# So-bonkers/Detecting-Convolutional-Codes-Via-Markovian-Statistics

Hardware: AMD Instinct MI355X
Metric: MC trials/sec at N=1e5, rate-1/2 m=6 pair, 1/2/4/8 GPUs; Pd match vs CPU (higher is better)
Workload: dtype u32 bit-planes (metrics, four planes of the 64 states) + f64 (log-likelihood sums)

## Files before the change

__graft_entry__.py:

```python
import importlib.util
import os
import subprocess
import sys

ROOT = os.path.dirname(os.path.abspath(__file__))
PKG_DIR = os.path.join(ROOT, "detecting-convolutional-codes-via-markovian-statistics_amd")
PKG_NAME = "dccvm_amd"


def load_package():
    if PKG_NAME in sys.modules:
        return sys.modules[PKG_NAME]
    spec = importlib.util.spec_from_file_location(
        PKG_NAME, os.path.join(PKG_DIR, "__init__.py"), submodule_search_locations=[PKG_DIR])
    mod = importlib.util.module_from_spec(spec)
    sys.modules[PKG_NAME] = mod
    spec.loader.exec_module(mod)
    return mod


def build() -> None:
    jobs = str(min(16, os.cpu_count() or 4))
    subprocess.check_call(["make", "-j", jobs, "-C", os.path.join(PKG_DIR, "csrc")])
    subprocess.check_call(["make", "-C", os.path.join(ROOT, "oracle")])
# ... 2 lines not shown
    prebuild_jit(pkg, lib)


def prebuild_jit(pkg, lib, arch="gfx950"):
    import ctypes
    jit_dir = os.path.join(PKG_DIR, "lib", "jit")
    so_time = os.path.getmtime(os.path.join(PKG_DIR, "lib", "libcvd.so"))
    if os.path.isdir(jit_dir):
        old = [f for f in os.listdir(jit_dir) if f.endswith(".co")]
        if any(os.path.getmtime(os.path.join(jit_dir, f)) < so_time for f in old):
            for f in old:
                os.remove(os.path.join(jit_dir, f))
    for name, cc in pkg.CONFIG_CODES.items():
        code = pkg.Code(cc["gen1"], cc["m"], cc["k"], cc["n"])
        n = ctypes.c_int32(0)
        rc = lib.cvd_jit_prebuild(code.c, arch.encode(), jit_dir.encode(), ctypes.byref(n))
        if rc != 0:
            print(f"jit prebuild of {name} failed: {lib.cvd_last_error().decode(errors='replace')}", file=sys.stderr)


def smoke() -> None:
    if ROOT not in sys.path:
        sys.path.insert(0, ROOT)
    pkg = load_package()
    from oracle import restatement as R
    k, n, m = 1, 2, 2
    g1 = [[[1, 1, 1]], [[1, 0, 1]]]
    g2 = [[[1, 0, 1]], [[1, 1, 1]]]
    N, p, seed, trials = 200, 0.1, 123, 64
    det = pkg.Detector(k, n, m, g1, device=0)
    model = det.model(p, learn_len=None, learn_burn=200, laplace=1.0, seed=seed)
    res = det.run_trials(model, g1, g2, N, p, seed, 0, trials, return_sums=True)
    states, transitions, all_r = R.enumerate_markov_states_allzero(g1, m, k, n)
# ... 36 lines not shown
```

detecting-convolutional-codes-via-markovian-statistics_amd/_lib.py:

```python
import ctypes
import os

import torch

_HERE = os.path.dirname(os.path.abspath(__file__))
LIB_PATH = os.environ.get("CVD_LIB_PATH") or os.path.join(_HERE, "lib", "libcvd.so")
ABI_VERSION = 11

PATH_AUTO, PATH_TABLE, PATH_EXPLICIT, PATH_EXPLICIT_GENERIC, PATH_EXPLICIT_ORBIT, PATH_EXPLICIT_BUTTERFLY = 0, 1, 2, 3, 4, 5
DETECT_EARLY_DECISION = 0x100
CAPTURE_LSB, CAPTURE_MSB, CAPTURE_BYTES = 0, 1, 2
CAPTURE_FORMATS = {"lsb": CAPTURE_LSB, "msb": CAPTURE_MSB, "bytes": CAPTURE_BYTES}


class CvdError(RuntimeError):
    """Raised when a libcvd call returns a negative status."""


class cvd_code(ctypes.Structure):
    _fields_ = [("k", ctypes.c_int32), ("n", ctypes.c_int32), ("m", ctypes.c_int32),
                ("taps", ctypes.POINTER(ctypes.c_uint8))]


class cvd_learn_params(ctypes.Structure):
# ... 73 lines not shown
    "cvd_mc_workspace_bytes": (ctypes.c_int64, [ctypes.POINTER(cvd_code), ctypes.c_int64, ctypes.c_int64]),
    "cvd_mc_run": (ctypes.c_int, [ctypes.c_void_p, ctypes.POINTER(cvd_code), ctypes.POINTER(cvd_code),
                                  ctypes.c_double, ctypes.c_int64, ctypes.c_uint64, ctypes.c_int64,
                                  ctypes.c_int64, ctypes.c_int64, ctypes.c_void_p, ctypes.c_void_p,
                                  ctypes.c_int32, ctypes.c_void_p]),
    "cvd_mc_grid_workspace_bytes": (ctypes.c_int64, [ctypes.c_void_p, ctypes.c_int32, ctypes.POINTER(cvd_code),
                                                     ctypes.c_void_p, ctypes.c_int32, ctypes.c_int64, ctypes.c_int32]),
    "cvd_mc_run_grid": (ctypes.c_int, [ctypes.c_void_p, ctypes.POINTER(cvd_code), ctypes.POINTER(cvd_code),
                                       ctypes.c_void_p, ctypes.c_int32, ctypes.c_void_p, ctypes.c_int32,
                                       ctypes.c_uint64, ctypes.c_int64, ctypes.c_int64, ctypes.c_int64,
                                       ctypes.c_void_p, ctypes.c_void_p, ctypes.c_int32, ctypes.c_void_p]),
    "cvd_model_device_error": (ctypes.c_int, [ctypes.c_void_p, ctypes.POINTER(ctypes.c_int32)]),
    "cvd_chunk_last": (ctypes.c_int, [ctypes.POINTER(ctypes.c_int64)]),
    "cvd_jit_prebuild": (ctypes.c_int, [ctypes.POINTER(cvd_code), ctypes.c_char_p, ctypes.c_char_p,
                                        ctypes.POINTER(ctypes.c_int32)]),
    "cvd_mc_fused": (ctypes.c_int, [ctypes.c_void_p, ctypes.POINTER(cvd_code), ctypes.POINTER(cvd_code),
                                    ctypes.c_double, ctypes.c_int64, ctypes.c_uint64, ctypes.c_int64,
                                    ctypes.c_int64, ctypes.c_void_p, ctypes.c_void_p, ctypes.c_int32,
                                    ctypes.c_void_p]),
    "cvd_parity_detect": (ctypes.c_int, [ctypes.c_void_p, ctypes.c_int32, ctypes.c_int64, ctypes.c_int64,
                                         ctypes.c_int64, ctypes.c_void_p, ctypes.c_int32, ctypes.c_double,
                                         ctypes.c_void_p, ctypes.c_void_p, ctypes.c_void_p]),
    "cvd_parity_sweep_workspace_bytes": (ctypes.c_int64, [ctypes.c_int32, ctypes.c_int32, ctypes.c_int32]),
    "cvd_parity_sweep": (ctypes.c_int, [ctypes.c_void_p, ctypes.c_int64, ctypes.c_int32, ctypes.c_int32,
                                        ctypes.c_int32, ctypes.c_int64, ctypes.c_int64, ctypes.c_int32,
                                        ctypes.c_void_p, ctypes.c_void_p, ctypes.c_void_p]),
    "cvd_viterbi_workspace_bytes": (ctypes.c_int64, [ctypes.c_int32, ctypes.c_int32, ctypes.c_int64, ctypes.c_int32]),
    "cvd_viterbi_decode": (ctypes.c_int, [ctypes.POINTER(cvd_code), ctypes.c_void_p, ctypes.c_int64, ctypes.c_int32,
                                          ctypes.c_int64, ctypes.c_int64, ctypes.c_int32, ctypes.c_int32,
                                          ctypes.c_int32, ctypes.c_void_p, ctypes.c_void_p, ctypes.c_void_p,
# ... 77 lines not shown
```

detecting-convolutional-codes-via-markovian-statistics_amd/csrc/cvd_host.cpp:

```cpp
#include <atomic>
#include <chrono>
#include <functional>
#include <map>
#include <mutex>
#include <thread>
#include <tuple>
#include <cstdlib>
#include <exception>
#include <cstdio>
#include <algorithm>
#include <cmath>
#include <cstring>
#include <memory>
#include <new>
#include <stdexcept>
#include <string>
#include <unordered_map>
#include <vector>

#include <sys/stat.h>
#include <unistd.h>

#include "../../include/cvd.h"
#include "cvd_internal.h"
// ... 1060 lines not shown
  const auto t0 = std::chrono::steady_clock::now();
  const int rc = model_create(dec, prm, device, stream, out, &st);
  st.seconds = std::chrono::duration<double>(std::chrono::steady_clock::now() - t0).count();
  if (stats_out) {
    stats_out[0] = st.seconds;
    stats_out[1] = (double)st.mismatched_blocks;
    stats_out[2] = (double)st.fix_passes;
    stats_out[3] = (double)st.sequential_blocks;
    stats_out[4] = (double)st.hash_attempts;
    stats_out[5] = (double)st.host_fallback;
    stats_out[6] = st.sequential_seconds;
  }
  return rc;
}

extern "C" int cvd_jit_prebuild(const cvd_code* dec, const char* arch, const char* dir, int32_t* n_built) {
  CVD_TRY
  if (!dec || !arch || !dir || !n_built) { set_error("null argument"); return CVD_E_INVALID; }
  *n_built = 0;
  cvd_model Mo;
  int rc = parse_code(dec, Mo.dec);
  if (rc) return rc;
  const Tabs T = make_tabs(Mo.dec);
  build_bmp(Mo, T);
  if (!Mo.k1b_ok || !bitslice_preferred(Mo)) return CVD_OK;
  const std::string vs[] = {
      rtc_variant_defs(kBsPfLog2Bits >= 20 ? 1024 : 512, false, kFilterPatBitsLds, true, true, kBsPfLog2Bits),
      rtc_variant_defs(1024, true, kFilterPatBitsLds, true, false, kBsPfLog2Bits),
      rtc_variant_defs(512, true, kFilterPatBitsLds, true, false, kBsPfLog2Bits)};
  std::vector<std::thread> th;
  std::vector<int> res(3, 0);
  std::vector<std::string> errs(3);
  for (int i = 0; i < 3; ++i)
    th.emplace_back([&, i] {
      res[i] = rtc_prebuild(Mo.dec.m, Mo.bfly_x, vs[i].c_str(), arch, dir);
      if (res[i]) errs[i] = last_error_copy();
    });
  for (auto& t : th) t.join();
  for (int i = 0; i < 3; ++i) {
    if (res[i]) { set_error(errs[i]); return CVD_E_UNSUPPORTED; }
    ++*n_built;
  }
  return CVD_OK;
  CVD_CATCH
}

extern "C" int cvd_model_info_get(const cvd_model* Mo, cvd_model_info* info) {
  if (!Mo || !info) { set_error("null argument"); return CVD_E_INVALID; }
  info->kind = Mo->kind;
  info->k = Mo->dec.k; info->n = Mo->dec.n; info->m = Mo->dec.m;
  info->S = Mo->S;
  info->n_rows = Mo->n_rows;
  info->learn_len_eff = Mo->learn_len_eff;
  info->hash_capacity = Mo->hcap;
  info->max_probe = Mo->max_probe;
  info->device = Mo->device;
  info->logp1_unseen = Mo->logp1_unseen;
  info->explicit_kernel = explicit_kernel_of(*Mo);
  info->mc_fused = mc_fused_preferred(*Mo) ? 1 : 0;
// ... 65 lines not shown
```

detecting-convolutional-codes-via-markovian-statistics_amd/csrc/cvd_internal.h:

```cpp
#pragma once
#include <stdint.h>

#include <array>
#include <string>
#include <vector>

#include "cvd_common.h"
#include "cvd_keys.h"

struct cvd_code;

struct cvd_model {
  cvd::CodeDesc dec;
  int32_t kind = 0;
  int64_t S = 0;
  int64_t learn_len_eff = 0;
  double laplace = 1.0;
  double logp1_unseen = 0.0;
  double lp_min = 0.0;
  std::vector<double> ltref;

  int64_t n_rows = 0;
  std::vector<uint8_t> keys;
  std::vector<double> logp1;
// ... 34 lines not shown
  int32_t slot0 = 0;
  std::vector<uint32_t> bmp;
  bool k1_ok = false;
  uint32_t repmap = 0, swmap = 0;
  std::vector<uint32_t> bmk1;
  bool k1b_ok = false;
  uint32_t bfly_uni = 0;
  uint32_t bfly_even[4] = {0, 0, 0, 0};
  uint64_t bfly_x = 0;
  void* rtc_fn = nullptr;
  void* rtc_fn_multi = nullptr;
  int rtc_block = 256;
  bool rtc_ldsf = false;
  bool rtc_pf = false;
  int64_t rtc_persist_grid = 0;
  std::string jit_error;
  std::vector<uint32_t> bfly;

  int device = -1;
  uint32_t* d_rec = nullptr;
  double* d_logp1 = nullptr;
  double* d_ltref = nullptr;
  uint32_t* d_filt = nullptr;
  uint32_t* d_filt_lds = nullptr;
  uint32_t* d_hkey = nullptr;
  uint32_t* d_hrow = nullptr;
  uint32_t* d_drow = nullptr;
  uint32_t* d_dkey = nullptr;
  uint32_t* d_t2 = nullptr;
  uint32_t* d_t2c = nullptr;
// ... 34 lines not shown
bool ldsf_preferred(const cvd_model& M);
bool ldsf_wanted(const cvd_model& M);
int launch_mc_fused(const cvd_model& M, const CodeDesc& e1, const CodeDesc& e2, uint32_t k0, uint32_t k1,
                    uint32_t tag, uint64_t thr, int64_t N, int64_t trial_begin, int64_t T, double* d_sums,
                    int64_t* d_counts, void* stream, bool early);
int launch_detect_explicit(const cvd_model& M, const uint32_t* d_r, int64_t N, int64_t nseq,
                           int64_t n_h1, double* d_sums, int64_t* d_counts, uint8_t* d_trace,
                           void* stream, int variant, bool early = false);
constexpr int kExplicitBest = 0, kExplicitOrbit = 1, kExplicitGeneric = 2, kExplicitButterfly = 3;
int upload_model(cvd_model& M, int device);
int explicit_kernel_of(const cvd_model& M);
int check_device(const cvd_model& M);
int rtc_k1b_function(int device, int m, uint64_t xm, const char* variant_defs, void** fn_out,
                     void** fn_multi_out = nullptr);
std::string rtc_variant_defs(int block, bool ldsf, int patbits, bool bs, bool pf, int pf_log2, bool slot3 = false);
int rtc_prebuild(int m, uint64_t xm, const char* variant_defs, const char* arch, const char* dir);
void free_model_device(cvd_model& M);
bool explicit_supported(int m, int k, int n);
bool bitslice_preferred(const cvd_model& M);
int64_t multi_variant(const cvd_model& M);
int64_t persist_seqs(const cvd_model& M);
extern std::array<int64_t, 4> ck_last;
int64_t persist_grid(const cvd_model& M, int64_t nseq);

struct LearnStats {
  int64_t mismatched_blocks = 0;
  int64_t fix_passes = 0;
  int64_t sequential_blocks = 0;
  int64_t hash_attempts = 0;
  double seconds = 0.0;
// ... 33 lines not shown
```

detecting-convolutional-codes-via-markovian-statistics_amd/csrc/cvd_k1s.h:

```cpp
#pragma once

#ifndef CVD_K1B_BITSLICE
#define CVD_K1B_BITSLICE 0
#endif

namespace cvd_dev {

constexpr int kBsSlotShift = 6;
constexpr int kBsRecWord = 48;
#ifndef CVD_K1S_SLOT3
#define CVD_K1S_SLOT3 0
#endif
constexpr bool kSlot3 = CVD_K1S_SLOT3 != 0;
template <int PH>
__device__ __forceinline__ constexpr uint32_t bs_img_off() {
  return kSlot3 ? 128u * (PH / 2) + 32u * (PH % 2) : 32u * PH;
}
template <int PH>
__device__ __forceinline__ constexpr uint32_t bs_rec_off() {
  return kSlot3 ? 128u * (PH / 2) + 64u : 4u * kBsRecWord;
}
constexpr int kBsDkeyWords = 48;
constexpr int kBsEarlyGroups = 21;
#ifndef CVD_K1S_ABL
// ... 11 lines not shown
constexpr bool kK1sT2 = CVD_K1S_T2 != 0;
#ifndef CVD_K1S_MIDPOS
#define CVD_K1S_MIDPOS 0
#endif
#ifndef CVD_K1S_AMASK
#define CVD_K1S_AMASK 1
#endif
#ifndef CVD_K1S_VMASK
#define CVD_K1S_VMASK 0
#endif
#ifndef CVD_K1S_PADV
#define CVD_K1S_PADV 0
#endif
#ifndef CVD_K1S_CK
#define CVD_K1S_CK 1
#endif
#ifndef CVD_K1S_R16
#define CVD_K1S_R16 1
#endif
constexpr bool kR16 = CVD_K1S_R16 != 0;
__device__ __forceinline__ uint32_t word_off16(uint32_t rp) { return kR16 ? rp : 16u * rp; }
__device__ __forceinline__ uint32_t word_param(uint32_t r) { return kR16 ? 16u * r : r; }

#ifndef CVD_K1S_NT_STREAM
#define CVD_K1S_NT_STREAM 1
#endif
#ifndef CVD_WALK_BUF
#define CVD_WALK_BUF 0
#endif
static_assert(CVD_WALK_BUF >= 0 && CVD_WALK_BUF <= 2, "CVD_WALK_BUF: 0, 1 or 2");
// ... 690 lines not shown
  p[0] = make_uint4(R[0][0], R[0][1], R[0][2], R[0][3]);
  p[1] = make_uint4(R[1][0], R[1][1], R[1][2], R[1][3]);
}

template <uint64_t XM, bool kCk = false>
__device__ __forceinline__ void k1s_wave(const ExpArgs& a, int64_t gw, const double* s_lt, int32_t ck_j = 0) {
  constexpr bool kUni = xm_uni<6, XM>();
  if (a.walk || (a.mix && !kCk)) {
    const int64_t half = ((a.nseq + 63) / 64 + 1) / 2, k = gw >> 1;
    if (gw < 2 * half) gw = ((gw ^ (gw >> 2)) & 1) ? half + k : k;
  }
  const int64_t qwave = gw * 64;
  const int64_t q = qwave + lane_id();
  const bool valid = q < a.nseq;
  const uint64_t vmask = __ballot(valid), hmask = __ballot(q < a.n_h1);
  if (a.walk && vmask != 0u && hmask == vmask) {
    k1s_walk<XM>(a, qwave, vmask, s_lt);
    return;
  }
  if ((CVD_WALK_ABL & 4) && a.walk) return;
  double lp = 0.0, lr = 0.0;
  if (valid) {
    uint32_t R[2][4] = {{0u, 0u, 0u, 0u}, {0u, 0u, 0u, 0u}};
    double lpu = a.lp_unseen;
    asm volatile("" : "+v"(lpu));
    const int64_t N = a.N, nwords = (N + 15) / 16;
    const size_t cstride = (size_t)a.nseq * 4;
    constexpr bool ck = kCk;
    int64_t t_begin = 0, t_sum = 0, t_end = N;
    if (ck) {
      t_sum = (int64_t)ck_j * a.ck_len;
      t_end = min(N, t_sum + (int64_t)a.ck_len);
      t_begin = max((int64_t)0, t_sum - (int64_t)a.ck_warm);
// ... 237 lines not shown
```

detecting-convolutional-codes-via-markovian-statistics_amd/csrc/cvd_kernels.hip:

```cpp
#include <hip/hip_runtime.h>

#include <algorithm>
#include <atomic>
#include <cstdlib>
#include <string>

#include "../../include/cvd.h"
#include "cvd_common.h"
#include "cvd_internal.h"
#include "cvd_device.h"

using namespace cvd;

#define HIP_CHECK(x)                                                                      \
  do {                                                                                    \
    hipError_t e_ = (x);                                                                  \
    if (e_ != hipSuccess) {                                                               \
      set_error(std::string("HIP error '") + hipGetErrorString(e_) + "' at " #x);          \
      return CVD_E_HIP;                                                                   \
    }                                                                                     \
  } while (0)

using namespace cvd_dev;

// ... 546 lines not shown
                         int64_t nwords, uint32_t (&out4)[4]) {
    if (a->thr_all) {
#pragma unroll
      for (int g = 0; g < 4; ++g) F[g] = kValid;
    } else if (a->thr_lo) {
      noise_exchange<CVD_FUSED_XCHG_SPLIT>(*a, su, sm, seq, (uint32_t)w4, U, F, keys());
    } else {
#pragma unroll
      for (int g = 0; g < 4; ++g) F[g] = 0u;
    }
#pragma unroll
    for (int g = 0; g < 4; ++g) out4[g] = w4 + g < nwords ? encode(w4 + g, F[g]) : 0u;
  }
};

template <int k, int n, int kT>
__global__ __launch_bounds__(kBlock) void gen_fast_kernel(GenArgs a) {
  constexpr int SPW = 32 / n;
  static_assert(k >= 1 && k <= 2 && SPW * k <= 32, "gen_fast_kernel: shape");
  const int64_t li = (int64_t)blockIdx.x * kBlock + threadIdx.x;
  const bool lane_ok = li < a.count;
  const int64_t q = a.q0 + li;
  const uint64_t sid = (uint64_t)(a.seq_base + li * a.seq_stride);
#if CVD_GEN_SEQ_LDS
  __shared__ NoiseLds noise_lds[kBlock / 64];
  NoiseLds& nl = noise_lds[threadIdx.x / 64];
  nl.slo[lane_id()] = (uint32_t)sid;
  nl.nhi[lane_id()] = ctr_hi(sid, kKindNoise);
  wave_lds_sync();
  auto seq = [&](uint32_t l) { return make_uint2(nl.slo[l], nl.nhi[l]); };
  uint32_t* const su = nl.u;
  uint32_t* const sm = nl.m;
#else
  __shared__ uint32_t xchg[kBlock / 64][128];
  uint32_t* const su = xchg[threadIdx.x / 64];
  uint32_t* const sm = su + 64;
  const int64_t li0 = (int64_t)blockIdx.x * kBlock + (int64_t)__builtin_amdgcn_readfirstlane(threadIdx.x & ~63u);
  const uint64_t s0 = (uint64_t)(a.seq_base + li0 * a.seq_stride), sstr = (uint64_t)a.seq_stride;
  auto seq = [&](uint32_t l) {
    const uint64_t s = s0 + (uint64_t)l * sstr;
    return make_uint2((uint32_t)s, ctr_hi(s, kKindNoise));
  };
#endif
  const int64_t nwords = (a.N + SPW - 1) / SPW;
  const int64_t nw4 = (nwords + 3) & ~(int64_t)3;
  ChunkEncoder<k, n, kT, CVD_GEN_VKEYS != 0> enc;
  enc.init(&a, sid);
  const int64_t nchunks = nw4 >> 2, seg = gridDim.y;
  const int64_t c0 = nchunks * blockIdx.y / seg, c1 = nchunks * (blockIdx.y + 1) / seg;
  if (c0 > 0 && 4 * c0 <= nwords) enc.seek(4 * c0);
  for (int64_t w4 = 4 * c0; w4 < 4 * c1; w4 += 4) {
    bool live[4];
#pragma unroll
    for (int g = 0; g < 4; ++g) live[g] = lane_ok && w4 + g < nwords;
    uint32_t out4[4];
    enc.chunk(su, sm, seq, w4, live, nwords, out4);
    if (lane_ok)
      *reinterpret_cast<uint4*>(a.r + chunk_index(w4 >> 2, a.pitch, q)) = make_uint4(out4[0], out4[1], out4[2], out4[3]);
  }
}

// ... 735 lines not shown
  return a;
}

bool gen_fast_ok(const CodeDesc& enc) {
  return !std::getenv("CVD_GEN_GENERIC") && enc.m <= kMaxM && enc.k <= 2 &&
         (enc.m + enc.k - 1) / enc.k + 32 / std::max(enc.n, 1) <= 32;
}

int tap_slots(int ntap) {
  if (ntap <= 0 || std::getenv("CVD_GEN_TAP_LOOP")) return 0;
  for (int t : {3, 4, 5, 6, 8})
    if (ntap <= t) return t;
  return 0;
}

template <int k, int n>
void (*gen_fast_variant(int kt))(GenArgs) {
  if constexpr (k == 2 && !CVD_GEN_K2_STRIDE3) return gen_fast_kernel<k, n, 0>;
  switch (kt) {
    case 3: return gen_fast_kernel<k, n, 3>;
    case 4: return gen_fast_kernel<k, n, 4>;
    case 5: return gen_fast_kernel<k, n, 5>;
    case 6: return gen_fast_kernel<k, n, 6>;
    case 8: return gen_fast_kernel<k, n, 8>;
    default: return gen_fast_kernel<k, n, 0>;
  }
}
}

int cvd::launch_generate(const CodeDesc& enc, uint32_t k0, uint32_t k1, uint32_t tag, uint64_t thr,
                         int64_t N, int random_input, int64_t seq_base, int64_t seq_stride,
                         uint32_t* d_r, int64_t pitch, int64_t q0, int64_t count, void* stream) {
  if (count <= 0 || N <= 0) return CVD_OK;
  GenArgs a = gen_args(enc, k0, k1, tag, thr, N, random_input);
  a.seq_base = seq_base; a.seq_stride = seq_stride;
  a.pitch = pitch; a.q0 = q0; a.count = count; a.r = d_r;
  const unsigned grid = (unsigned)((count + kBlock - 1) / kBlock);
  const bool fast = gen_fast_ok(enc);
  auto kern = gen_kernel<0, 0>;
  dim3 gdim(grid);
  if (fast) {
    const int64_t nchunks = (((N + 32 / enc.n - 1) / (32 / enc.n)) + 3) / 4;
    const int64_t waves = (count + 63) / 64;
    const int64_t seg = std::max<int64_t>(1, std::min<int64_t>((16 * 1024 + waves - 1) / waves, nchunks / 16));
    gdim.y = (unsigned)std::min<int64_t>(seg, 65535);
  }
  const int kt = tap_slots(a.ntap);
  if (fast && enc.k == 1 && enc.n == 2) kern = gen_fast_variant<1, 2>(kt);
  else if (fast && enc.k == 1 && enc.n == 3) kern = gen_fast_variant<1, 3>(kt);
  else if (fast && enc.k == 2 && enc.n == 3) kern = gen_fast_variant<2, 3>(kt);
  else if (enc.k == 1 && enc.n == 2) kern = gen_kernel<1, 2>;
  else if (enc.k == 1 && enc.n == 3) kern = gen_kernel<1, 3>;
  else if (enc.k == 2 && enc.n == 3) kern = gen_kernel<2, 3>;
  hipLaunchKernelGGL(kern, gdim, dim3(kBlock), 0, (hipStream_t)stream, a);
  HIP_CHECK(hipGetLastError());
  return CVD_OK;
}

namespace {
bool table_lr(const cvd_model& M) {
  const int64_t SR = M.S * ((int64_t)1 << M.dec.n);
  return SR * 18 <= 32 * 1024 && !std::getenv("CVD_TABLE_NOLR");
}
// ... 203 lines not shown
  if (a.t2 && which == CVD_KERNEL_BUTTERFLY_RTC && M.rtc_bs && M.rtc_ldsf && M.rtc_t2c) {
    a.t2 = M.d_t2c;
    a.t2c = 1;
    a.vtab = M.d_vtab;
    a.nvtab = (int32_t)M.h_vtab.size();
    a.vtab_off = (uint32_t)(M.fcap * sizeof(uint32_t));
  }
  a.walk = which == CVD_KERNEL_BUTTERFLY_RTC && !d_trace && N < ((int64_t)1 << 31) && M.d_dkey && walk_preferred(M, a.early);
  a.walk_wmin = env_i("CVD_WALK_WMIN", 48);
  a.walk_amin = env_i("CVD_WALK_AMIN", 4);
  a.walk_burst = a.t2 ? std::max(1, std::min(7, env_i("CVD_WALK_BURST", 7)))
                      : std::max(1, std::min(16, env_i("CVD_WALK_BURST", 16)));
  return a;
}

int cvd::launch_detect_explicit(const cvd_model& M, const uint32_t* d_r, int64_t N, int64_t nseq,
                                int64_t n_h1, double* d_sums, int64_t* d_counts, uint8_t* d_trace,
                                void* stream, int variant, bool early) {
  ExpKernel kern = nullptr;
  const uint32_t* bmp = nullptr;
  const int which = select_explicit(M, variant, &kern, &bmp, d_trace != nullptr);
  if (which == CVD_KERNEL_NONE || !M.d_filt || !bmp) {
    set_error("explicit path: unsupported code shape (m,k,n)");
    return CVD_E_UNSUPPORTED;
  }
  if (nseq <= 0) return CVD_OK;
  ExpArgs a = exp_args(M, which, d_r, N, nseq, n_h1, d_sums, d_counts, d_trace, bmp, early);
  const unsigned grid = (unsigned)((nseq + kBlock - 1) / kBlock);
  if (which == CVD_KERNEL_BUTTERFLY_RTC) {
    void* args[] = {&a};
    const unsigned blk = (unsigned)M.rtc_block;
    unsigned rgrid = (unsigned)((nseq + blk - 1) / blk);
    const unsigned lds = rtc_dyn_lds(M);
    if (const int64_t pgrid = persist_grid(M, nseq); pgrid > 0) {
      HIP_CHECK(hipMallocAsync((void**)&a.wq, sizeof(uint32_t), (hipStream_t)stream));
      HIP_CHECK(hipMemsetAsync(a.wq, 0, sizeof(uint32_t), (hipStream_t)stream));
      rgrid = (unsigned)pgrid;
    }
    HIP_CHECK(hipModuleLaunchKernel((hipFunction_t)M.rtc_fn, rgrid, 1, 1, blk, 1, 1, lds,
                                    (hipStream_t)stream, args, nullptr));
    if (a.wq) HIP_CHECK(hipFreeAsync(a.wq, (hipStream_t)stream));
    return CVD_OK;
  }
  hipLaunchKernelGGL(kern, dim3(grid), dim3(kBlock), 0, (hipStream_t)stream, a);
  HIP_CHECK(hipGetLastError());
  return CVD_OK;
}

static int launch_multi(const cvd_model* const* models, int32_t i0, int32_t i1, const uint32_t* const* d_r,
                        int64_t N, const int64_t* nseq, const int64_t* n_h1, double* const* d_sums,
                        int64_t* const* d_counts, void* stream, bool early) {
  const cvd_model& M0 = *models[i0];
  MultiArgs ma;
  ma.nm = 0;
  uint32_t blocks = 0;
  const unsigned blk = (unsigned)M0.rtc_block;
  for (int32_t i = i0; i < i1; ++i) {
    const cvd_model& M = *models[i];
    if (nseq[i] <= 0) continue;
    const int64_t nb = (nseq[i] + blk - 1) / blk;
    if ((int64_t)blocks + nb > (int64_t)UINT32_MAX) { set_error("multi-model launch: grid too large"); return CVD_E_INVALID; }
    ma.a[ma.nm] = exp_args(M, CVD_KERNEL_BUTTERFLY_RTC, d_r[i], N, nseq[i], n_h1[i], d_sums ? d_sums[i] : nullptr,
                           d_counts[i], nullptr, M.d_bfly, early);
    blocks += (uint32_t)nb;
    ma.blk_end[ma.nm] = blocks;
    ++ma.nm;
  }
  if (ma.nm == 0) return CVD_OK;
  for (int j = ma.nm; j < kMultiMax; ++j) ma.blk_end[j] = blocks;
  void* args[] = {&ma};
  const unsigned lds = rtc_dyn_lds(M0);
  HIP_CHECK(hipModuleLaunchKernel((hipFunction_t)M0.rtc_fn_multi, blocks, 1, 1, blk, 1, 1, lds, (hipStream_t)stream,
                                  args, nullptr));
  return CVD_OK;
}

std::array<int64_t, 4> cvd::ck_last = {0, 0, 0, 0};
struct CkPlan {
  int32_t C = 0, L = 0, W = 0;
};
static int64_t round_up192(int64_t x) { return (x + 191) / 192 * 192; }
static bool ck_plan(const cvd_model& M, int64_t N, int64_t nseq_total, CkPlan* P) {
  const int mode = env_i("CVD_CHUNK", -1);
  if (mode == 0 || !M.rtc_fn || !M.rtc_bs || N <= 0 || N >= ((int64_t)1 << 30) || nseq_total <= 0) return false;
  const int64_t W = round_up192(std::max(0, env_i("CVD_CHUNK_WARM", 1152)));
  const int64_t slots = std::max<int64_t>(1, M.rtc_persist_grid) * (M.rtc_block / 64);
  const int64_t waves = (nseq_total + 63) / 64;
// ... 185 lines not shown
    if ((rc = dev_copy(M.d_bfilt_lds, M.h_bfilt_lds))) return rc;
    if ((rc = dev_directory(M.d_bkey, M.h_bkey_rows, M.h_bkey_slot, M.bhcap, M.bs_slot_w, 0u))) return rc;
    if ((rc = dev_copy(M.d_bdkey, M.h_bdkey))) return rc;
    if ((rc = dev_copy(M.d_bpf, M.h_bpf))) return rc;
    if ((rc = dev_copy(M.d_bmp, M.bmp))) return rc;
    if ((rc = dev_copy(M.d_bmk1, M.bmk1))) return rc;
    if ((rc = dev_copy(M.d_bfly, M.bfly))) return rc;
  }
  HIP_CHECK(hipMalloc((void**)&M.d_err, sizeof(int32_t)));
  HIP_CHECK(hipMemset(M.d_err, 0, sizeof(int32_t)));
  M.device = device;
  M.lp_min = M.kind == 1 ? M.logp1_unseen : 0.0;
  for (double v : M.logp1) M.lp_min = std::min(M.lp_min, v);
  M.rtc_fn = nullptr;
  M.rtc_fn_multi = nullptr;
  M.jit_error.clear();
  M.rtc_ldsf = M.k1b_ok && M.hcap > 0 && ldsf_preferred(M);
  M.rtc_bs = false;
  M.rtc_pf = false;
  for (int attempt = M.bs && M.d_bkey ? 0 : 1; attempt < 2 && M.k1b_ok && M.hcap > 0; ++attempt) {
    const bool bs = attempt == 0;
    const bool pf = bs && !M.rtc_ldsf && M.d_bpf != nullptr;
    M.rtc_block = pf ? (M.bs_pf_log2 >= 20 ? 1024 : 512) : env_i("CVD_K1B_BLOCK", M.rtc_ldsf ? (M.fcap > ((int64_t)1 << 14) ? 1024 : 512) : kBlock);
    if (M.rtc_block != 256 && M.rtc_block != 512 && M.rtc_block != 1024) M.rtc_block = kBlock;
    const int patbits = M.rtc_ldsf ? kFilterPatBitsLds : bs ? M.bs_pat_bits : kFilterPatBits;
    const std::string vdefs = rtc_variant_defs(M.rtc_block, M.rtc_ldsf, patbits, bs, pf, M.bs_pf_log2, M.bs_slot_w == 96);
    if (rtc_k1b_function(device, M.dec.m, M.bfly_x, vdefs.c_str(), &M.rtc_fn, &M.rtc_fn_multi) == 0) {
      M.rtc_bs = bs;
      M.rtc_pf = pf;
      M.jit_error.clear();
      break;
    }
    M.rtc_fn = nullptr;
    M.rtc_fn_multi = nullptr;
    M.jit_error = last_error_copy();
  }
  if (!M.rtc_fn) {
    M.rtc_ldsf = false;
    M.rtc_block = kBlock;
  }
  M.rtc_t2c = false;
  if (M.rtc_fn && M.rtc_bs && M.rtc_ldsf && M.d_t2c && M.d_vtab) {
    int st = 0, mx = 0;
    if (hipFuncGetAttribute(&st, HIP_FUNC_ATTRIBUTE_SHARED_SIZE_BYTES, (hipFunction_t)M.rtc_fn) == hipSuccess &&
// ... 18 lines not shown
  int cur = 0;
  (void)hipGetDevice(&cur);
  (void)hipSetDevice(M.device);
  void* ptrs[] = {M.d_rec, M.d_logp1, M.d_ltref, M.d_filt, M.d_filt_lds, M.d_hkey, M.d_hrow, M.d_drow, M.d_dkey, M.d_t2,
                  M.d_t2c, M.d_vtab, M.d_bmp,
                  M.d_bmk1, M.d_bfly, M.d_err, M.d_bfilt, M.d_bfilt_lds, M.d_bkey, M.d_bdkey, M.d_bpf};
  for (void* p : ptrs)
    if (p) (void)hipFree(p);
  M.d_rec = nullptr; M.d_logp1 = nullptr; M.d_ltref = nullptr;
  M.d_filt = nullptr; M.d_filt_lds = nullptr; M.d_hkey = nullptr; M.d_hrow = nullptr; M.d_drow = nullptr; M.d_dkey = nullptr; M.d_t2 = nullptr;
  M.d_t2c = nullptr; M.d_vtab = nullptr; M.rtc_t2c = false;
  M.d_bfilt = nullptr; M.d_bfilt_lds = nullptr; M.d_bkey = nullptr; M.d_bdkey = nullptr; M.d_bpf = nullptr;
  M.rtc_persist_grid = 0;
  M.rtc_bs = false;
  M.rtc_pf = false;
  M.d_bmp = nullptr;
  M.d_bmk1 = nullptr;
  M.d_bfly = nullptr;
  M.d_err = nullptr;
  M.rtc_fn = nullptr;
  M.rtc_fn_multi = nullptr;
  M.device = -1;
  (void)hipSetDevice(cur);
}


namespace {
int parse_code_dev(const cvd_code* c, CodeDesc& d) {
  if (!c || !c->taps || c->k < 1 || c->k > kMaxK || c->n < 1 || c->n > kMaxN || c->m < 1 || c->m > kMaxM) {
    set_error("bad code description");
// ... 400 lines not shown
```

detecting-convolutional-codes-via-markovian-statistics_amd/csrc/cvd_rtc.cpp:

```cpp
#include <hip/hip_runtime.h>
#include <hip/hiprtc.h>
#include <dlfcn.h>
#include <fcntl.h>
#include <spawn.h>
#include <sys/file.h>
#include <sys/stat.h>
#include <sys/wait.h>
#include <unistd.h>

#include <cstdio>
#include <cstdlib>
#include <fstream>
#include <map>
#include <mutex>
#include <sstream>
#include <string>
#include <tuple>
#include <vector>

#include "cvd_internal.h"

#include "cvd_rtc_src.inc"

extern char** environ;
// ... 41 lines not shown
void cache_store(const std::string& path, const std::vector<char>& code) {
  const std::string tmp = path + ".tmp." + std::to_string(::getpid());
  {
    std::ofstream f(tmp, std::ios::binary);
    if (!f) return;
    f.write(code.data(), (std::streamsize)code.size());
    if (!f) { ::unlink(tmp.c_str()); return; }
  }
  if (::rename(tmp.c_str(), path.c_str()) != 0) ::unlink(tmp.c_str());
}

const char* kClangFlags[] = {"-O3", "-std=c++17", "-ffp-contract=off",
                             "-mllvm", "--amdgpu-sched-strategy=max-ilp"};

std::string entry_source(int m, uint64_t xm) {
  char entry[640];
  std::snprintf(entry, sizeof(entry),
                "\nextern \"C\" __global__ __launch_bounds__(cvd_dev::kK1bBlock, cvd_dev::kK1bWavesPerSimd)\n"
                "void cvd_k1b_spec(cvd_dev::ExpArgs a) { cvd_dev::k1b_spec_entry<%d, 0x%016llxull>(a); }\n"
                "extern \"C\" __global__ __launch_bounds__(cvd_dev::kK1bBlock, cvd_dev::kK1bWavesPerSimd)\n"
                "void cvd_k1b_spec_multi(cvd_dev::MultiArgs a) { cvd_dev::k1b_spec_multi_entry<%d, 0x%016llxull>(a); }\n",
                m, (unsigned long long)xm, m, (unsigned long long)xm);
  return entry;
}

bool file_exists(const std::string& p) {
  struct stat st;
  return ::stat(p.c_str(), &st) == 0;
}

std::string find_clang();
std::string object_name(const std::string& src, const std::string& arch, const std::string& all_defs) {
  std::string keytxt = src + "\n" + arch + "\n" + find_clang() + "\n" + all_defs;
  for (const char* f : kClangFlags) keytxt += std::string("\n") + f;
  char name[64];
// ... 110 lines not shown
}

int cvd::rtc_k1b_function(int device, int m, uint64_t xm, const char* variant_defs, void** fn_out,
                          void** fn_multi_out) {
  *fn_out = nullptr;
  if (fn_multi_out) *fn_multi_out = nullptr;
  if (const char* e = std::getenv("CVD_NO_JIT"))
    if (e[0] && e[0] != '0') { set_error("JIT: disabled by CVD_NO_JIT"); return -1; }
  std::lock_guard<std::mutex> lock(g_mu);
  std::string env_defs;
  if (const char* e = std::getenv("CVD_JIT_DEFINES")) {
    std::istringstream ds(e);
    std::string t;
    while (ds >> t)
      if (t.rfind("-DCVD_K1B_BLOCK", 0) != 0 && t.rfind("-DCVD_K1B_LDSF", 0) != 0 &&
          t.rfind("-DCVD_FILTER_PAT_BITS", 0) != 0 && t.rfind("-DCVD_K1S_PF", 0) != 0)
        env_defs += " " + t;
  }
  const std::string all_defs = std::string(variant_defs ? variant_defs : "") + env_defs;
  const auto key = std::make_tuple(device, m, xm, all_defs);
  auto it = g_cache.find(key);
  if (it != g_cache.end()) {
    *fn_out = (void*)it->second.first;
    if (fn_multi_out) *fn_multi_out = (void*)it->second.second;
    return 0;
  }
  hipDeviceProp_t prop;
  if (hipGetDeviceProperties(&prop, device) != hipSuccess) { set_error("JIT: device properties"); return -1; }
  std::string arch = prop.gcnArchName;
  const size_t colon = arch.find(':');
  if (colon != std::string::npos) arch = arch.substr(0, colon);
// ... 78 lines not shown
```

detecting-convolutional-codes-via-markovian-statistics_amd/csrc/spec_resource.py:

```python
#!/usr/bin/env python3
import os
import subprocess
import sys
import tempfile

HERE = os.path.dirname(os.path.abspath(__file__))
sys.path.insert(0, os.path.dirname(os.path.dirname(HERE)))


def code_constant(cfg):
    from __graft_entry__ import load_package
    pkg = load_package()
    cc = pkg.CONFIG_CODES[cfg]
    out, _ = pkg.Code(cc["gen1"], cc["m"], cc["k"], cc["n"]).tables()
    return cc["m"], sum(int(out[j, 0]) << (2 * j) for j in range((1 << cc["m"]) // 2))


def main():
    args = sys.argv[1:]
    isa = None
    if "--isa" in args:
        i = args.index("--isa")
        isa = args[i + 1]
        del args[i:i + 2]
    defs = [x for x in args if x.startswith("-")]
    rest = [x for x in args if not x.startswith("-")]
    m, xm = code_constant(rest[0] if rest else "m6")
    clang = os.environ.get("CVD_JIT_CLANG", "/opt/rocm/lib/llvm/bin/clang++")
    with tempfile.TemporaryDirectory() as d:
        src = os.path.join(d, "k1b_spec.hip")
        with open(src, "w") as f:
            f.write('#include <hip/hip_runtime.h>\n#include "cvd_device.h"\n'
                    'extern "C" __global__ __launch_bounds__(cvd_dev::kK1bBlock, cvd_dev::kK1bWavesPerSimd)\n'
                    f'void cvd_k1b_spec(cvd_dev::ExpArgs a) {{ cvd_dev::k1b_spec_entry<{m}, 0x{xm:016x}ull>(a); }}\n'
                    'extern "C" __global__ __launch_bounds__(cvd_dev::kK1bBlock, cvd_dev::kK1bWavesPerSimd)\n'
                    f'void cvd_k1b_spec_multi(cvd_dev::MultiArgs a) {{ cvd_dev::k1b_spec_multi_entry<{m}, 0x{xm:016x}ull>(a); }}\n')
        base = [clang, "-x", "hip", "--offload-arch=gfx950", "--offload-device-only", "--no-gpu-bundle-output",
                "-O3", "-std=c++17", "-ffp-contract=off", "-mllvm", "--amdgpu-sched-strategy=max-ilp",
                "-I", HERE, *defs]
        r = subprocess.run(base + ["-Rpass-analysis=kernel-resource-usage", "-c", src, "-o",
                                   os.path.join(d, "k.co")], capture_output=True, text=True)
        for line in r.stderr.splitlines():
            if "remark" in line or "error" in line:
                print(line.split("remark: ")[-1])
        if r.returncode:
            sys.exit(r.returncode)
        if isa:
            subprocess.run(base + ["-S", src, "-o", isa], check=True)
            print("ISA written to", isa)

# ... 4 lines not shown
```

include/cvd.h:

```cpp
#ifndef CVD_H
#define CVD_H
#include <stdint.h>

#ifdef __cplusplus
extern "C" {
#endif

#define CVD_ABI_VERSION 11

#define CVD_OK 0
#define CVD_E_INVALID -1
#define CVD_E_UNSUPPORTED -2
#define CVD_E_CAPACITY -3
#define CVD_E_HIP -4
#define CVD_E_STATE -5

typedef struct cvd_code {
  int32_t k, n, m;
  const uint8_t* taps;
} cvd_code;

typedef struct cvd_learn_params {
  double p;
  int64_t learn_len;
// ... 99 lines not shown
               int64_t batch, void* d_work, int64_t* d_counts, int32_t path, void* stream);


int64_t cvd_mc_grid_workspace_bytes(const cvd_model* const* models, int32_t np, const cvd_code* enc1,
                                    const int64_t* N, int32_t nN, int64_t batch, int32_t path);
int cvd_mc_run_grid(const cvd_model* const* models, const cvd_code* enc1, const cvd_code* enc2,
                    const double* p, int32_t np, const int64_t* N, int32_t nN, uint64_t seed,
                    int64_t trial_begin, int64_t trial_end, int64_t batch, void* d_work,
                    int64_t* d_counts, int32_t path, void* stream);

int cvd_model_device_error(cvd_model* model, int32_t* flags_out);

int cvd_chunk_last(int64_t* out4);

int cvd_jit_prebuild(const cvd_code* dec, const char* arch, const char* dir, int32_t* n_built);

int cvd_mc_fused(const cvd_model* model, const cvd_code* enc1, const cvd_code* enc2, double p, int64_t N,
                 uint64_t seed, int64_t trial_begin, int64_t trial_end, double* d_sums, int64_t* d_counts,
                 int32_t flags, void* stream);

int cvd_allreduce_counts(int64_t* const* d_counts, int64_t len, int32_t ndev, const int32_t* devices,
                         void* const* streams);
#define CVD_COMM_ID_BYTES 128
typedef struct cvd_comm cvd_comm;
int cvd_comm_unique_id(uint8_t* id_out );
int cvd_comm_init(const uint8_t* id, int32_t nranks, int32_t rank, int32_t device, cvd_comm** out);
int cvd_comm_allreduce_counts(cvd_comm* comm, int64_t* d_counts, int64_t len, void* stream);
void cvd_comm_destroy(cvd_comm* comm);

int cvd_parity_detect(const uint32_t* d_r, int32_t n, int64_t N, int64_t nseq, int64_t n_h1,
// ... 68 lines not shown
```

Before: 1.488 million.

## Compile no-walk bitslice detector variant and pick smaller generator form beside persistent kernel

When the walk path is not preferred, the JIT-compiled bitslice detector is now built with the walk branch compiled out and a pinned waves-per-EU attribute, which should cut register pressure and raise occupancy. A walking variant is compiled lazily when a launch needs it, and both variants are prebuilt. Separately, the generator kernel for rate-1/2 codes switches to a non-vector-keys form when a persistent detector kernel from another stream is still running on the same device, so the two can share the GPU better. The cost is extra JIT variants, host-side event bookkeeping and mutex locking, and a generator choice that depends on runtime timing.

```diff
diff --git a/__graft_entry__.py b/__graft_entry__.py
--- a/__graft_entry__.py
+++ b/__graft_entry__.py
@@ -40,9 +40,10 @@
     for name, cc in pkg.CONFIG_CODES.items():
         code = pkg.Code(cc["gen1"], cc["m"], cc["k"], cc["n"])
         n = ctypes.c_int32(0)
-        rc = lib.cvd_jit_prebuild(code.c, arch.encode(), jit_dir.encode(), ctypes.byref(n))
-        if rc != 0:
-            print(f"jit prebuild of {name} failed: {lib.cvd_last_error().decode(errors='replace')}", file=sys.stderr)
+        for fn in (lib.cvd_jit_prebuild, lib.cvd_jit_prebuild_walk):
+            rc = fn(code.c, arch.encode(), jit_dir.encode(), ctypes.byref(n))
+            if rc != 0:
+                print(f"jit prebuild of {name} failed: {lib.cvd_last_error().decode(errors='replace')}", file=sys.stderr)
 
 
 def smoke() -> None:
diff --git a/detecting-convolutional-codes-via-markovian-statistics_amd/_lib.py b/detecting-convolutional-codes-via-markovian-statistics_amd/_lib.py
--- a/detecting-convolutional-codes-via-markovian-statistics_amd/_lib.py
+++ b/detecting-convolutional-codes-via-markovian-statistics_amd/_lib.py
@@ -111,6 +111,8 @@
     "cvd_chunk_last": (ctypes.c_int, [ctypes.POINTER(ctypes.c_int64)]),
     "cvd_jit_prebuild": (ctypes.c_int, [ctypes.POINTER(cvd_code), ctypes.c_char_p, ctypes.c_char_p,
                                         ctypes.POINTER(ctypes.c_int32)]),
+    "cvd_jit_prebuild_walk": (ctypes.c_int, [ctypes.POINTER(cvd_code), ctypes.c_char_p, ctypes.c_char_p,
+                                             ctypes.POINTER(ctypes.c_int32)]),
     "cvd_mc_fused": (ctypes.c_int, [ctypes.c_void_p, ctypes.POINTER(cvd_code), ctypes.POINTER(cvd_code),
                                     ctypes.c_double, ctypes.c_int64, ctypes.c_uint64, ctypes.c_int64,
                                     ctypes.c_int64, ctypes.c_void_p, ctypes.c_void_p, ctypes.c_int32,
diff --git a/detecting-convolutional-codes-via-markovian-statistics_amd/csrc/cvd_host.cpp b/detecting-convolutional-codes-via-markovian-statistics_amd/csrc/cvd_host.cpp
--- a/detecting-convolutional-codes-via-markovian-statistics_amd/csrc/cvd_host.cpp
+++ b/detecting-convolutional-codes-via-markovian-statistics_amd/csrc/cvd_host.cpp
@@ -1098,7 +1098,7 @@
   return rc;
 }
 
-extern "C" int cvd_jit_prebuild(const cvd_code* dec, const char* arch, const char* dir, int32_t* n_built) {
+static int jit_prebuild(const cvd_code* dec, const char* arch, const char* dir, int32_t* n_built, bool walk) {
   CVD_TRY
   if (!dec || !arch || !dir || !n_built) { set_error("null argument"); return CVD_E_INVALID; }
   *n_built = 0;
@@ -1108,10 +1108,11 @@
   const Tabs T = make_tabs(Mo.dec);
   build_bmp(Mo, T);
   if (!Mo.k1b_ok || !bitslice_preferred(Mo)) return CVD_OK;
+  const std::string nw = walk ? "" : kNoWalkDef;
   const std::string vs[] = {
-      rtc_variant_defs(kBsPfLog2Bits >= 20 ? 1024 : 512, false, kFilterPatBitsLds, true, true, kBsPfLog2Bits),
-      rtc_variant_defs(1024, true, kFilterPatBitsLds, true, false, kBsPfLog2Bits),
-      rtc_variant_defs(512, true, kFilterPatBitsLds, true, false, kBsPfLog2Bits)};
+      rtc_variant_defs(kBsPfLog2Bits >= 20 ? 1024 : 512, false, kFilterPatBitsLds, true, true, kBsPfLog2Bits) + nw,
+      rtc_variant_defs(1024, true, kFilterPatBitsLds, true, false, kBsPfLog2Bits) + nw,
+      rtc_variant_defs(512, true, kFilterPatBitsLds, true, false, kBsPfLog2Bits) + nw};
   std::vector<std::thread> th;
   std::vector<int> res(3, 0);
   std::vector<std::string> errs(3);
@@ -1127,6 +1128,12 @@
   }
   return CVD_OK;
   CVD_CATCH
+}
+extern "C" int cvd_jit_prebuild(const cvd_code* dec, const char* arch, const char* dir, int32_t* n_built) {
+  return jit_prebuild(dec, arch, dir, n_built, false);
+}
+extern "C" int cvd_jit_prebuild_walk(const cvd_code* dec, const char* arch, const char* dir, int32_t* n_built) {
+  return jit_prebuild(dec, arch, dir, n_built, true);
 }
 
 extern "C" int cvd_model_info_get(const cvd_model* Mo, cvd_model_info* info) {
diff --git a/detecting-convolutional-codes-via-markovian-statistics_amd/csrc/cvd_internal.h b/detecting-convolutional-codes-via-markovian-statistics_amd/csrc/cvd_internal.h
--- a/detecting-convolutional-codes-via-markovian-statistics_amd/csrc/cvd_internal.h
+++ b/detecting-convolutional-codes-via-markovian-statistics_amd/csrc/cvd_internal.h
@@ -72,6 +72,10 @@
   bool rtc_ldsf = false;
   bool rtc_pf = false;
   int64_t rtc_persist_grid = 0;
+  bool rtc_nowalk = false;
+  std::string rtc_walk_defs;
+  mutable void* rtc_fn_walk = nullptr;
+  mutable void* rtc_fn_multi_walk = nullptr;
   std::string jit_error;
   std::vector<uint32_t> bfly;
 
@@ -136,6 +140,7 @@
 int rtc_k1b_function(int device, int m, uint64_t xm, const char* variant_defs, void** fn_out,
                      void** fn_multi_out = nullptr);
 std::string rtc_variant_defs(int block, bool ldsf, int patbits, bool bs, bool pf, int pf_log2, bool slot3 = false);
+constexpr const char* kNoWalkDef = " -DCVD_K1S_WALK=0";
 int rtc_prebuild(int m, uint64_t xm, const char* variant_defs, const char* arch, const char* dir);
 void free_model_device(cvd_model& M);
 bool explicit_supported(int m, int k, int n);
diff --git a/detecting-convolutional-codes-via-markovian-statistics_amd/csrc/cvd_k1s.h b/detecting-convolutional-codes-via-markovian-statistics_amd/csrc/cvd_k1s.h
--- a/detecting-convolutional-codes-via-markovian-statistics_amd/csrc/cvd_k1s.h
+++ b/detecting-convolutional-codes-via-markovian-statistics_amd/csrc/cvd_k1s.h
@@ -49,6 +49,14 @@
 #endif
 #ifndef CVD_K1S_CK
 #define CVD_K1S_CK 1
+#endif
+#ifndef CVD_K1S_WALK
+#define CVD_K1S_WALK 1
+#endif
+#if CVD_K1B_BITSLICE && !CVD_K1S_WALK
+#define CVD_K1B_ENTRY_ATTR __attribute__((amdgpu_waves_per_eu(CVD_K1B_WAVES, CVD_K1B_WAVES)))
+#else
+#define CVD_K1B_ENTRY_ATTR
 #endif
 #ifndef CVD_K1S_R16
 #define CVD_K1S_R16 1
@@ -769,9 +777,11 @@
   const int64_t q = qwave + lane_id();
   const bool valid = q < a.nseq;
   const uint64_t vmask = __ballot(valid), hmask = __ballot(q < a.n_h1);
-  if (a.walk && vmask != 0u && hmask == vmask) {
-    k1s_walk<XM>(a, qwave, vmask, s_lt);
-    return;
+  if constexpr (CVD_K1S_WALK != 0) {
+    if (a.walk && vmask != 0u && hmask == vmask) {
+      k1s_walk<XM>(a, qwave, vmask, s_lt);
+      return;
+    }
   }
   if ((CVD_WALK_ABL & 4) && a.walk) return;
   double lp = 0.0, lr = 0.0;
diff --git a/detecting-convolutional-codes-via-markovian-statistics_amd/csrc/cvd_kernels.hip b/detecting-convolutional-codes-via-markovian-statistics_amd/csrc/cvd_kernels.hip
--- a/detecting-convolutional-codes-via-markovian-statistics_amd/csrc/cvd_kernels.hip
+++ b/detecting-convolutional-codes-via-markovian-statistics_amd/csrc/cvd_kernels.hip
@@ -3,6 +3,9 @@
 #include <algorithm>
 #include <atomic>
 #include <cstdlib>
+#include <cstring>
+#include <map>
+#include <mutex>
 #include <string>
 
 #include "../../include/cvd.h"
@@ -584,7 +587,7 @@
   }
 };
 
-template <int k, int n, int kT>
+template <int k, int n, int kT, bool kVK = CVD_GEN_VKEYS != 0>
 __global__ __launch_bounds__(kBlock) void gen_fast_kernel(GenArgs a) {
   constexpr int SPW = 32 / n;
   static_assert(k >= 1 && k <= 2 && SPW * k <= 32, "gen_fast_kernel: shape");
@@ -614,7 +617,7 @@
 #endif
   const int64_t nwords = (a.N + SPW - 1) / SPW;
   const int64_t nw4 = (nwords + 3) & ~(int64_t)3;
-  ChunkEncoder<k, n, kT, CVD_GEN_VKEYS != 0> enc;
+  ChunkEncoder<k, n, kT, kVK> enc;
   enc.init(&a, sid);
   const int64_t nchunks = nw4 >> 2, seg = gridDim.y;
   const int64_t c0 = nchunks * blockIdx.y / seg, c1 = nchunks * (blockIdx.y + 1) / seg;
@@ -1380,9 +1383,71 @@
   return 0;
 }
 
+struct PersistMark {
+  hipEvent_t ev = nullptr;
+  hipStream_t stream = nullptr;
+  bool set = false;
+};
+std::mutex g_persist_mu;
+std::map<int, PersistMark> g_persist;
+
+void persist_mark(hipStream_t stream) {
+  int dev = 0;
+  hipStreamCaptureStatus cap = hipStreamCaptureStatusNone;
+  if (hipGetDevice(&dev) != hipSuccess) return;
+  if (hipStreamIsCapturing(stream, &cap) != hipSuccess || cap != hipStreamCaptureStatusNone) return;
+  std::lock_guard<std::mutex> lock(g_persist_mu);
+  PersistMark& m = g_persist[dev];
+  if (!m.ev && hipEventCreateWithFlags(&m.ev, hipEventDisableTiming) != hipSuccess) {
+    m.ev = nullptr;
+    return;
+  }
+  m.set = hipEventRecord(m.ev, stream) == hipSuccess;
+  m.stream = stream;
+}
+
+bool persist_beside(hipStream_t stream) {
+  int dev = 0;
+  if (hipGetDevice(&dev) != hipSuccess) return false;
+  hipStreamCaptureStatus cap = hipStreamCaptureStatusNone;
+  if (hipStreamIsCapturing(stream, &cap) != hipSuccess) {
+    (void)hipGetLastError();
+    return false;
+  }
+  if (cap != hipStreamCaptureStatusNone) return false;
+  std::lock_guard<std::mutex> lock(g_persist_mu);
+  auto it = g_persist.find(dev);
+  if (it == g_persist.end() || !it->second.set || it->second.stream == stream) return false;
+  const hipError_t q = hipEventQuery(it->second.ev);
+  if (q != hipErrorNotReady) {
+    if (q != hipSuccess) (void)hipGetLastError();
+    it->second.set = false;
+    return false;
+  }
+  return true;
+}
+
+bool gen_small_form(hipStream_t stream) {
+  if (const char* e = std::getenv("CVD_GEN_FORM")) {
+    if (!std::strcmp(e, "small")) return true;
+    if (!std::strcmp(e, "fast")) return false;
+  }
+  return persist_beside(stream);
+}
+
 template <int k, int n>
-void (*gen_fast_variant(int kt))(GenArgs) {
+void (*gen_fast_variant(int kt, bool small = false))(GenArgs) {
   if constexpr (k == 2 && !CVD_GEN_K2_STRIDE3) return gen_fast_kernel<k, n, 0>;
+  if constexpr (k == 1 && n == 2 && CVD_GEN_VKEYS != 0) {
+    if (small) switch (kt) {
+      case 3: return gen_fast_kernel<k, n, 3, false>;
+      case 4: return gen_fast_kernel<k, n, 4, false>;
+      case 5: return gen_fast_kernel<k, n, 5, false>;
+      case 6: return gen_fast_kernel<k, n, 6, false>;
+      case 8: return gen_fast_kernel<k, n, 8, false>;
+      default: return gen_fast_kernel<k, n, 0, false>;
+    }
+  }
   switch (kt) {
     case 3: return gen_fast_kernel<k, n, 3>;
     case 4: return gen_fast_kernel<k, n, 4>;
@@ -1412,7 +1477,7 @@
     gdim.y = (unsigned)std::min<int64_t>(seg, 65535);
   }
   const int kt = tap_slots(a.ntap);
-  if (fast && enc.k == 1 && enc.n == 2) kern = gen_fast_variant<1, 2>(kt);
+  if (fast && enc.k == 1 && enc.n == 2) kern = gen_fast_variant<1, 2>(kt, gen_small_form((hipStream_t)stream));
   else if (fast && enc.k == 1 && enc.n == 3) kern = gen_fast_variant<1, 3>(kt);
   else if (fast && enc.k == 2 && enc.n == 3) kern = gen_fast_variant<2, 3>(kt);
   else if (enc.k == 1 && enc.n == 2) kern = gen_kernel<1, 2>;
@@ -1646,6 +1711,26 @@
   return a;
 }
 
+static int rtc_entries(const cvd_model& M, bool walk, void** fn, void** fn_multi) {
+  *fn = M.rtc_fn;
+  if (fn_multi) *fn_multi = M.rtc_fn_multi;
+  if (!walk || !M.rtc_nowalk) return CVD_OK;
+  static std::mutex mu;
+  std::lock_guard<std::mutex> lock(mu);
+  if (!M.rtc_fn_walk &&
+      rtc_k1b_function(M.device, M.dec.m, M.bfly_x, M.rtc_walk_defs.c_str(), &M.rtc_fn_walk, &M.rtc_fn_multi_walk) != 0) {
+    M.rtc_fn_walk = nullptr;
+    M.rtc_fn_multi_walk = nullptr;
+    return CVD_E_UNSUPPORTED;
+  }
+  *fn = M.rtc_fn_walk;
+  if (fn_multi) {
+    if (!M.rtc_fn_multi_walk) { set_error("walking variant without the multi-model entry"); return CVD_E_UNSUPPORTED; }
+    *fn_multi = M.rtc_fn_multi_walk;
+  }
+  return CVD_OK;
+}
+
 int cvd::launch_detect_explicit(const cvd_model& M, const uint32_t* d_r, int64_t N, int64_t nseq,
                                 int64_t n_h1, double* d_sums, int64_t* d_counts, uint8_t* d_trace,
                                 void* stream, int variant, bool early) {
@@ -1661,6 +1746,8 @@
   const unsigned grid = (unsigned)((nseq + kBlock - 1) / kBlock);
   if (which == CVD_KERNEL_BUTTERFLY_RTC) {
     void* args[] = {&a};
+    void* fn = nullptr;
+    if (const int rc = rtc_entries(M, a.walk != 0, &fn, nullptr)) return rc;
     const unsigned blk = (unsigned)M.rtc_block;
     unsigned rgrid = (unsigned)((nseq + blk - 1) / blk);
     const unsigned lds = rtc_dyn_lds(M);
@@ -1669,9 +1756,12 @@
       HIP_CHECK(hipMemsetAsync(a.wq, 0, sizeof(uint32_t), (hipStream_t)stream));
       rgrid = (unsigned)pgrid;
     }
-    HIP_CHECK(hipModuleLaunchKernel((hipFunction_t)M.rtc_fn, rgrid, 1, 1, blk, 1, 1, lds,
+    HIP_CHECK(hipModuleLaunchKernel((hipFunction_t)fn, rgrid, 1, 1, blk, 1, 1, lds,
                                     (hipStream_t)stream, args, nullptr));
-    if (a.wq) HIP_CHECK(hipFreeAsync(a.wq, (hipStream_t)stream));
+    if (a.wq) {
+      HIP_CHECK(hipFreeAsync(a.wq, (hipStream_t)stream));
+      if (M.rtc_bs) persist_mark((hipStream_t)stream);
+    }
     return CVD_OK;
   }
   hipLaunchKernelGGL(kern, dim3(grid), dim3(kBlock), 0, (hipStream_t)stream, a);
@@ -1702,7 +1792,11 @@
   for (int j = ma.nm; j < kMultiMax; ++j) ma.blk_end[j] = blocks;
   void* args[] = {&ma};
   const unsigned lds = rtc_dyn_lds(M0);
-  HIP_CHECK(hipModuleLaunchKernel((hipFunction_t)M0.rtc_fn_multi, blocks, 1, 1, blk, 1, 1, lds, (hipStream_t)stream,
+  bool walks = false;
+  for (int j = 0; j < ma.nm; ++j) walks = walks || ma.a[j].walk != 0;
+  void *fn = nullptr, *fnm = nullptr;
+  if (const int rc = rtc_entries(M0, walks, &fn, &fnm)) return rc;
+  HIP_CHECK(hipModuleLaunchKernel((hipFunction_t)fnm, blocks, 1, 1, blk, 1, 1, lds, (hipStream_t)stream,
                                   args, nullptr));
   return CVD_OK;
 }
@@ -1918,6 +2012,9 @@
   for (double v : M.logp1) M.lp_min = std::min(M.lp_min, v);
   M.rtc_fn = nullptr;
   M.rtc_fn_multi = nullptr;
+  M.rtc_fn_walk = nullptr;
+  M.rtc_fn_multi_walk = nullptr;
+  M.rtc_nowalk = false;
   M.jit_error.clear();
   M.rtc_ldsf = M.k1b_ok && M.hcap > 0 && ldsf_preferred(M);
   M.rtc_bs = false;
@@ -1928,10 +2025,14 @@
     M.rtc_block = pf ? (M.bs_pf_log2 >= 20 ? 1024 : 512) : env_i("CVD_K1B_BLOCK", M.rtc_ldsf ? (M.fcap > ((int64_t)1 << 14) ? 1024 : 512) : kBlock);
     if (M.rtc_block != 256 && M.rtc_block != 512 && M.rtc_block != 1024) M.rtc_block = kBlock;
     const int patbits = M.rtc_ldsf ? kFilterPatBitsLds : bs ? M.bs_pat_bits : kFilterPatBits;
-    const std::string vdefs = rtc_variant_defs(M.rtc_block, M.rtc_ldsf, patbits, bs, pf, M.bs_pf_log2, M.bs_slot_w == 96);
+    const std::string wdefs = rtc_variant_defs(M.rtc_block, M.rtc_ldsf, patbits, bs, pf, M.bs_pf_log2, M.bs_slot_w == 96);
+    const bool nowalk = bs && !walk_preferred(M) && env_i("CVD_K1S_WALK_CODE", 0) == 0;
+    const std::string vdefs = wdefs + (nowalk ? kNoWalkDef : "");
     if (rtc_k1b_function(device, M.dec.m, M.bfly_x, vdefs.c_str(), &M.rtc_fn, &M.rtc_fn_multi) == 0) {
       M.rtc_bs = bs;
       M.rtc_pf = pf;
+      M.rtc_nowalk = nowalk;
+      M.rtc_walk_defs = wdefs;
       M.jit_error.clear();
       break;
     }
@@ -1980,6 +2081,9 @@
   M.rtc_persist_grid = 0;
   M.rtc_bs = false;
   M.rtc_pf = false;
+  M.rtc_nowalk = false;
+  M.rtc_fn_walk = nullptr;
+  M.rtc_fn_multi_walk = nullptr;
   M.d_bmp = nullptr;
   M.d_bmk1 = nullptr;
   M.d_bfly = nullptr;
diff --git a/detecting-convolutional-codes-via-markovian-statistics_amd/csrc/cvd_rtc.cpp b/detecting-convolutional-codes-via-markovian-statistics_amd/csrc/cvd_rtc.cpp
--- a/detecting-convolutional-codes-via-markovian-statistics_amd/csrc/cvd_rtc.cpp
+++ b/detecting-convolutional-codes-via-markovian-statistics_amd/csrc/cvd_rtc.cpp
@@ -79,11 +79,11 @@
                              "-mllvm", "--amdgpu-sched-strategy=max-ilp"};
 
 std::string entry_source(int m, uint64_t xm) {
-  char entry[640];
+  char entry[768];
   std::snprintf(entry, sizeof(entry),
-                "\nextern \"C\" __global__ __launch_bounds__(cvd_dev::kK1bBlock, cvd_dev::kK1bWavesPerSimd)\n"
+                "\nextern \"C\" __global__ CVD_K1B_ENTRY_ATTR __launch_bounds__(cvd_dev::kK1bBlock, cvd_dev::kK1bWavesPerSimd)\n"
                 "void cvd_k1b_spec(cvd_dev::ExpArgs a) { cvd_dev::k1b_spec_entry<%d, 0x%016llxull>(a); }\n"
-                "extern \"C\" __global__ __launch_bounds__(cvd_dev::kK1bBlock, cvd_dev::kK1bWavesPerSimd)\n"
+                "extern \"C\" __global__ CVD_K1B_ENTRY_ATTR __launch_bounds__(cvd_dev::kK1bBlock, cvd_dev::kK1bWavesPerSimd)\n"
                 "void cvd_k1b_spec_multi(cvd_dev::MultiArgs a) { cvd_dev::k1b_spec_multi_entry<%d, 0x%016llxull>(a); }\n",
                 m, (unsigned long long)xm, m, (unsigned long long)xm);
   return entry;
@@ -224,7 +224,8 @@
     std::string t;
     while (ds >> t)
       if (t.rfind("-DCVD_K1B_BLOCK", 0) != 0 && t.rfind("-DCVD_K1B_LDSF", 0) != 0 &&
-          t.rfind("-DCVD_FILTER_PAT_BITS", 0) != 0 && t.rfind("-DCVD_K1S_PF", 0) != 0)
+          t.rfind("-DCVD_FILTER_PAT_BITS", 0) != 0 && t.rfind("-DCVD_K1S_PF", 0) != 0 &&
+          t.rfind("-DCVD_K1S_WALK=", 0) != 0)
         env_defs += " " + t;
   }
   const std::string all_defs = std::string(variant_defs ? variant_defs : "") + env_defs;
diff --git a/detecting-convolutional-codes-via-markovian-statistics_amd/csrc/spec_resource.py b/detecting-convolutional-codes-via-markovian-statistics_amd/csrc/spec_resource.py
--- a/detecting-convolutional-codes-via-markovian-statistics_amd/csrc/spec_resource.py
+++ b/detecting-convolutional-codes-via-markovian-statistics_amd/csrc/spec_resource.py
@@ -31,9 +31,9 @@
         src = os.path.join(d, "k1b_spec.hip")
         with open(src, "w") as f:
             f.write('#include <hip/hip_runtime.h>\n#include "cvd_device.h"\n'
-                    'extern "C" __global__ __launch_bounds__(cvd_dev::kK1bBlock, cvd_dev::kK1bWavesPerSimd)\n'
+                    'extern "C" __global__ CVD_K1B_ENTRY_ATTR __launch_bounds__(cvd_dev::kK1bBlock, cvd_dev::kK1bWavesPerSimd)\n'
                     f'void cvd_k1b_spec(cvd_dev::ExpArgs a) {{ cvd_dev::k1b_spec_entry<{m}, 0x{xm:016x}ull>(a); }}\n'
-                    'extern "C" __global__ __launch_bounds__(cvd_dev::kK1bBlock, cvd_dev::kK1bWavesPerSimd)\n'
+                    'extern "C" __global__ CVD_K1B_ENTRY_ATTR __launch_bounds__(cvd_dev::kK1bBlock, cvd_dev::kK1bWavesPerSimd)\n'
                     f'void cvd_k1b_spec_multi(cvd_dev::MultiArgs a) {{ cvd_dev::k1b_spec_multi_entry<{m}, 0x{xm:016x}ull>(a); }}\n')
         base = [clang, "-x", "hip", "--offload-arch=gfx950", "--offload-device-only", "--no-gpu-bundle-output",
                 "-O3", "-std=c++17", "-ffp-contract=off", "-mllvm", "--amdgpu-sched-strategy=max-ilp",
diff --git a/include/cvd.h b/include/cvd.h
--- a/include/cvd.h
+++ b/include/cvd.h
@@ -137,6 +137,7 @@
 int cvd_chunk_last(int64_t* out4);
 
 int cvd_jit_prebuild(const cvd_code* dec, const char* arch, const char* dir, int32_t* n_built);
+int cvd_jit_prebuild_walk(const cvd_code* dec, const char* arch, const char* dir, int32_t* n_built);
 
 int cvd_mc_fused(const cvd_model* model, const cvd_code* enc1, const cvd_code* enc2, double p, int64_t N,
                  uint64_t seed, int64_t trial_begin, int64_t trial_end, double* d_sums, int64_t* d_counts,
```

Result: faster. 1.514 million, median of 6 (+1.7%).
